# maxwerhahn/Multi-pass-GAN

Hardware: AMD Instinct MI355X
Metric: volumes/sec (4x two-pass generator inference, 64^3->256^3 density-only) (higher is better)
Workload: dtype f16+2xbf6->f32

## Files before the change

multi-pass-gan_amd/csrc/mpgan_conv.h:

```cpp
#pragma once
#include "mpgan_internal.h"
#include "mpgan_mfma_dev.h"

namespace mpg::conv {

using namespace mpg::dev;

constexpr int TW = 32;
constexpr int TAPOFF_BYTES = 1024;
constexpr int epi_rowf(int nt) { return nt * 32 + 4; }

struct SegArgs {
    const char* x;
    const char* w;
    int cg_seg;
    int cg_total, g_off;
    int kh, kw, up;
    int cgc, nchunks, sc;
    int ih, iw;
    int pt, pl;
    int hs, ws;
    int np;
    int ni_img;
    int direct;
// ... 51 lines not shown

template <int NT, int PREC>
struct Pipe {
    static constexpr int WAVES = 4;
    static constexpr int NPL = (PREC == 3) ? 2 : 1;
    static constexpr int PT = (NT >= 3) ? 2 : 4;
    static constexpr int TH = 4 * PT;
    static constexpr int KS = (PREC == 3) ? ((NT == 4 || NT == 2) ? 1 : 2) : ((NT == 4 || NT == 2) ? 2 : 4);
    static constexpr int R = (NT == 3) ? 3 : 4;
    static constexpr int D = R - 1;
    static constexpr int WPLANE = KS * NT * 1024;
    static constexpr int WSTAGE = WPLANE * NPL;
    static constexpr int NI = WSTAGE / 4096;
    static constexpr int ROWF = epi_rowf(NT);
    static_assert(WSTAGE % 4096 == 0, "stage must be a whole number of 256 x 16-byte pieces");
};

template <int NT>
struct Pipe6 {
    static constexpr int WAVES = (NT == 1) ? 4 : 8;
    static constexpr int PT = 16 / WAVES;
    static constexpr int TH = 16;
    static constexpr int KS = 4;
    static constexpr int WF16 = KS * NT * 1024;
    static constexpr int WF6 = NT * 2048;
    static constexpr int WSTAGE = WF16 + 2 * WF6;
    static constexpr int R = 3;
    static constexpr int D = R - 1;
    static constexpr int NI = WSTAGE / (WAVES * 1024);
    static constexpr int ROWF = epi_rowf(NT);
    static_assert(WSTAGE % (WAVES * 1024) == 0, "stage must be a whole number of per-wave pieces");
};

template <int NT, int PT, bool D2S = false>
__device__ __forceinline__ void conv_epilogue(f32x16 (&acc)[PT][NT], const KArgs ap, char* smem, int n, int y0, int x0,
                                              int wave, int lane) {
    const auto& a = *ap;
    const KArgsD2S dp = reinterpret_cast<KArgsD2S>(ap);
    const int r = lane & 31;
    const int hh = lane >> 5;
    constexpr int ROWF = epi_rowf(NT);
    float* stg = reinterpret_cast<float*>(smem + TAPOFF_BYTES) + wave * (32 * ROWF);
    const int cg_out = (a.cout + 7) >> 3;
    const float unscale = a.in_amax != nullptr ? 1.f / mpg::pow2_scale(*a.in_amax) : 1.f;
#pragma unroll
    for (int pt = 0; pt < PT; ++pt) {
        const int py = y0 + PT * wave + pt;
        float ss = 0.f;
#pragma unroll
        for (int nt = 0; nt < NT; ++nt)
#pragma unroll
            for (int q4 = 0; q4 < 4; ++q4) {
                const int co0 = nt * 32 + 8 * q4 + 4 * hh;
                float b4[4] = {0.f, 0.f, 0.f, 0.f};
                if (a.bias != nullptr) {
#pragma unroll
                    for (int i = 0; i < 4; ++i)
                        if (co0 + i < a.cout) b4[i] = a.bias[co0 + i];
                }
#pragma unroll
                for (int i = 0; i < 4; ++i) {
                    float v = mpg::apply_act(acc[pt][nt][4 * q4 + i] * unscale + b4[i], a.act, a.leak);
                    if (co0 + i >= a.cout) v = 0.f;
                    acc[pt][nt][4 * q4 + i] = v;
                    ss += v * v;
                }
            }
        if (a.pn) {
            ss += __shfl_xor(ss, 32);
            const float sc = rsqrtf(ss / (float)a.cout + a.pn_eps);
#pragma unroll
            for (int nt = 0; nt < NT; ++nt)
#pragma unroll
                for (int i = 0; i < 16; ++i) acc[pt][nt][i] *= sc;
        }
        if (a.y == nullptr && a.post_add == nullptr) {
            const int npx = min(32, a.w - x0);
            if (py < a.h && r < npx && !(a.dbg & 2)) {
                const size_t plane_px = (size_t)a.h * a.w;
#pragma unroll
                for (int nt = 0; nt < NT; ++nt)
#pragma unroll
                    for (int qp = 0; qp < 2; ++qp) {
                        float v[8];
#pragma unroll
                        for (int i = 0; i < 4; ++i) {
                            typedef unsigned v2u_t __attribute__((ext_vector_type(2)));
                            const v2u_t sw = __builtin_amdgcn_permlane32_swap(__float_as_uint(acc[pt][nt][8 * qp + i]),
                                                                              __float_as_uint(acc[pt][nt][8 * qp + 4 + i]), false, false);
                            v[i] = __uint_as_float(sw[0]);
                            v[4 + i] = __uint_as_float(sw[1]);
                        }
                        const int cg = nt * 4 + 2 * qp + hh;
                        if (cg < cg_out) {
                            char* dst;
                            size_t plane_out = plane_px;
                            if constexpr (D2S) {
                                const D2SPos q = d2s_pos(dp, py, x0 + r, 8 * cg);
                                plane_out = 4 * plane_px;
                                dst = a.y_g8 + ((((size_t)n * dp->cg + (q.cc >> 3)) * 2) * plane_out + q.pix) * 16;
                            } else {
                                dst = a.y_g8 + ((((size_t)n * cg_out + cg) * 2) * plane_px + (size_t)py * a.w + x0 + r) * 16;
                            }
                            half8 hi, lo;
#pragma unroll
                            for (int j = 0; j < 8; ++j) {
                                hi[j] = (_Float16)v[j];
                                lo[j] = (_Float16)(v[j] - (float)hi[j]);
                            }
                            __builtin_nontemporal_store(hi, reinterpret_cast<half8*>(dst));
                            __builtin_nontemporal_store(lo, reinterpret_cast<half8*>(dst + plane_out * 16));
                        }
                    }
            }
            continue;
        }
#pragma unroll
        for (int nt = 0; nt < NT; ++nt)
#pragma unroll
            for (int q4 = 0; q4 < 4; ++q4) {
                const int co0 = nt * 32 + 8 * q4 + 4 * hh;
                *reinterpret_cast<float4*>(stg + r * ROWF + co0) =
                    make_float4(acc[pt][nt][4 * q4], acc[pt][nt][4 * q4 + 1], acc[pt][nt][4 * q4 + 2], acc[pt][nt][4 * q4 + 3]);
            }
        if (py < a.h && !(a.dbg & 2)) {
            const int npx = min(32, a.w - x0);
            const size_t pix0 = ((size_t)n * a.h + py) * a.w + x0;
            if (a.post_add != nullptr) {
                const float* pa = a.post_add + pix0 * a.pa_stride + a.pa_coff;
                for (int f = lane; f < npx * a.cout; f += 64) {
                    const int p = f / a.cout;
                    const int c = f - p * a.cout;
                    stg[p * ROWF + c] += pa[(size_t)p * a.pa_stride + c];
                }
            }
            if (D2S && a.y != nullptr) {
                float* img = a.y + (size_t)n * 4 * a.h * a.w * dp->cs;
                const int total = npx * a.cout;
                if (((dp->cs | dp->coff | a.cout) & 3) == 0) {
                    for (int f = lane * 4; f < total; f += 256) {
                        const int p = f / a.cout;
                        const int c = f - p * a.cout;
                        const D2SPos q = d2s_pos(dp, py, x0 + p, c);
                        *reinterpret_cast<float4*>(img + q.pix * dp->cs + q.cc) = *reinterpret_cast<const float4*>(stg + p * ROWF + c);
                    }
                } else {
                    for (int f = lane; f < total; f += 64) {
                        const int p = f / a.cout;
                        const int c = f - p * a.cout;
                        const D2SPos q = d2s_pos(dp, py, x0 + p, c);
                        img[q.pix * dp->cs + q.cc] = stg[p * ROWF + c];
                    }
                }
            } else if (a.y != nullptr) {
                float* dst = a.y + pix0 * a.cout;
                const int total = npx * a.cout;
                if ((a.cout & 3) == 0) {
                    for (int f = lane * 4; f < total; f += 256) {
                        const int p = f / a.cout;
                        const int c = f - p * a.cout;
                        *reinterpret_cast<float4*>(dst + f) = *reinterpret_cast<const float4*>(stg + p * ROWF + c);
                    }
                } else {
                    for (int f = lane; f < total; f += 64) {
                        const int p = f / a.cout;
                        dst[f] = stg[p * ROWF + (f - p * a.cout)];
                    }
                }
            }
            if (a.y_g8 != nullptr) {
                const size_t plane_px = (size_t)a.h * a.w;
                if (r < npx) {
                    for (int cg = hh; cg < cg_out; cg += 2) {
                        const float4 v0 = *reinterpret_cast<const float4*>(stg + r * ROWF + cg * 8);
                        const float4 v1 = *reinterpret_cast<const float4*>(stg + r * ROWF + cg * 8 + 4);
                        const float v[8] = {v0.x, v0.y, v0.z, v0.w, v1.x, v1.y, v1.z, v1.w};
                        char* dst;
                        size_t plane_out = plane_px;
                        if constexpr (D2S) {
                            const D2SPos q = d2s_pos(dp, py, x0 + r, 8 * cg);
                            plane_out = 4 * plane_px;
                            dst = a.y_g8 + ((((size_t)n * dp->cg + (q.cc >> 3)) * 2) * plane_out + q.pix) * 16;
                        } else {
                            dst = a.y_g8 + ((((size_t)n * cg_out + cg) * 2) * plane_px + (size_t)py * a.w + x0 + r) * 16;
                        }
                        half8 hi, lo;
#pragma unroll
                        for (int j = 0; j < 8; ++j) {
                            hi[j] = (_Float16)v[j];
                            lo[j] = (_Float16)(v[j] - (float)hi[j]);
                        }
                        __builtin_nontemporal_store(hi, reinterpret_cast<half8*>(dst));
                        __builtin_nontemporal_store(lo, reinterpret_cast<half8*>(dst + plane_out * 16));
                    }
                }
            }
        }
    }
}

struct Shape {
    int th;
    int ks;
    int waves;
// ... 27 lines not shown
```

multi-pass-gan_amd/csrc/mpgan_conv_f16.hip:

```cpp
#include "mpgan_conv.h"

using namespace mpg::conv;

namespace {

template <int NT, int PREC, bool D2S = false>
__global__ __launch_bounds__(256, (NT >= 2 ? 2 : 3)) void conv_mfma_kernel(const typename KernelArgs<D2S>::type a_unused) {
    extern __shared__ __attribute__((aligned(16))) char smem[];
    const KArgs ap = (KArgs)__builtin_amdgcn_kernarg_segment_ptr();
    const auto& a = *ap;
    using P = Pipe<NT, PREC>;
    constexpr int PT = P::PT, TH = P::TH, KS = P::KS, WPLANE = P::WPLANE, WSTAGE = P::WSTAGE;
    constexpr int NI = P::NI, R = P::R, D = P::D;

    int* tapoff = reinterpret_cast<int*>(smem);
    char* img_lds = smem + TAPOFF_BYTES;
    char* w_lds = img_lds + 2 * a.img_bytes;

    const int tid = threadIdx.x;
    const int lane = tid & 63;
    const int wave = tid >> 6;
    const int wave_u = __builtin_amdgcn_readfirstlane(wave);
    const int r = lane & 31;
    const int hh = lane >> 5;

    int bid = blockIdx.x;
    const int nblk = gridDim.x;
    if ((nblk & 7) == 0) bid = (bid & 7) * (nblk >> 3) + (bid >> 3);
    const int tx = bid % a.tiles_x;
    const int t2 = bid / a.tiles_x;
    const int ty = t2 % a.tiles_y;
    const int n = t2 / a.tiles_y;
    const int y0 = ty * TH, x0 = tx * TW;

    f32x16 acc[PT][NT];
#pragma unroll
    for (int pt = 0; pt < PT; ++pt)
#pragma unroll
        for (int nt = 0; nt < NT; ++nt)
#pragma unroll
            for (int i = 0; i < 16; ++i) acc[pt][nt][i] = 0.f;

    for (int s = 0; s < ((a.dbg & 1) ? 0 : a.nseg); ++s) {
        const auto& sg = ap->seg[s];
        const int CGC = sg.cgc;
        const int TG = sg.kh * sg.kw * CGC;
        const int plane_b = sg.np * 16;
        const int group_b = plane_b * 2;
        const int ppg = sg.np >> 6;

        for (int q = tid; q < sg.sc * KS * 2; q += 256) {
            int off = 0;
            if (q < TG) {
                const int tap = q / CGC;
                const int g = q - tap * CGC;
                const int dy = tap / sg.kw;
                const int dx = tap - dy * sg.kw;
                off = (dy * sg.iw + dx) * 16 + g * group_b;
            }
            tapoff[q] = off;
        }
        int pixb[PT];
#pragma unroll
        for (int pt = 0; pt < PT; ++pt) pixb[pt] = ((PT * wave + pt) * sg.iw + r) * 16;

        const size_t plane_px = (size_t)sg.hs * sg.ws;
        auto dma_image = [&](int chunk) {
            char* buf = img_lds + (chunk & 1) * a.img_bytes;
            for (int i = 0; i < sg.ni_img; ++i) {
                const int pc = 4 * i + wave_u;
                const int g = pc / (2 * ppg);
                const int rem = pc - g * 2 * ppg;
                const int pl = rem / ppg;
                const int p = (rem - pl * ppg) * 64 + lane;
                const int hy = p / sg.iw;
// ... 33 lines not shown
                const char* wb = w_lds + (gst % R) * WSTAGE;
#pragma unroll
                for (int ks = 0; ks < KS; ++ks) {
                    const int toff = tapoff[2 * (st * KS + ks) + hh];
                    half8 b_hi[PT], b_lo[PT], a_hi[NT], a_lo[NT];
#pragma unroll
                    for (int pt = 0; pt < PT; ++pt) {
                        b_hi[pt] = *reinterpret_cast<const half8*>(img + pixb[pt] + toff);
                        if (PREC == 3) b_lo[pt] = *reinterpret_cast<const half8*>(img + plane_b + pixb[pt] + toff);
                    }
#pragma unroll
                    for (int nt = 0; nt < NT; ++nt) {
                        a_hi[nt] = *reinterpret_cast<const half8*>(wb + ((ks * NT + nt) * 64 + lane) * 16);
                        if (PREC == 3)
                            a_lo[nt] = *reinterpret_cast<const half8*>(wb + WPLANE + ((ks * NT + nt) * 64 + lane) * 16);
                    }
#pragma unroll
                    for (int nt = 0; nt < NT; ++nt)
#pragma unroll
                        for (int pt = 0; pt < PT; ++pt) {
                            acc[pt][nt] = __builtin_amdgcn_mfma_f32_32x32x16_f16(a_hi[nt], b_hi[pt], acc[pt][nt], 0, 0, 0);
                            if (PREC == 3) {
                                acc[pt][nt] = __builtin_amdgcn_mfma_f32_32x32x16_f16(a_lo[nt], b_hi[pt], acc[pt][nt], 0, 0, 0);
                                acc[pt][nt] = __builtin_amdgcn_mfma_f32_32x32x16_f16(a_hi[nt], b_lo[pt], acc[pt][nt], 0, 0, 0);
                            }
                        }
                }
            }
        }
        asm volatile("s_waitcnt vmcnt(0)" ::: "memory");
        __syncthreads();
    }

    conv_epilogue<NT, PT, D2S>(acc, ap, smem, n, y0, x0, wave, lane);
}

template <bool D2S>
hipError_t launch(int prec, int nt, dim3 grid, size_t lds, hipStream_t st, const typename KernelArgs<D2S>::type& a) {
    const dim3 block(256);
    if (prec == MPG_PREC_F16X3) {
        switch (nt) {
            case 1: return mpg::launch_dyn_lds<conv_mfma_kernel<1, 3, D2S>>(grid, block, lds, st, a);
            case 2: return mpg::launch_dyn_lds<conv_mfma_kernel<2, 3, D2S>>(grid, block, lds, st, a);
            case 3: return mpg::launch_dyn_lds<conv_mfma_kernel<3, 3, D2S>>(grid, block, lds, st, a);
            default: return mpg::launch_dyn_lds<conv_mfma_kernel<4, 3, D2S>>(grid, block, lds, st, a);
        }
    }
    switch (nt) {
        case 1: return mpg::launch_dyn_lds<conv_mfma_kernel<1, 1, D2S>>(grid, block, lds, st, a);
        case 2: return mpg::launch_dyn_lds<conv_mfma_kernel<2, 1, D2S>>(grid, block, lds, st, a);
        case 3: return mpg::launch_dyn_lds<conv_mfma_kernel<3, 1, D2S>>(grid, block, lds, st, a);
        default: return mpg::launch_dyn_lds<conv_mfma_kernel<4, 1, D2S>>(grid, block, lds, st, a);
    }
}

}

hipError_t mpg::conv::launch_conv_f16(int prec, int nt, dim3 grid, size_t lds, hipStream_t st, const ConvArgs& a) {
    return launch<false>(prec, nt, grid, lds, st, a);
}
hipError_t mpg::conv::launch_conv_f16(int prec, int nt, dim3 grid, size_t lds, hipStream_t st, const ConvArgsD2S& a) {
    return launch<true>(prec, nt, grid, lds, st, a);
}
```

multi-pass-gan_amd/csrc/mpgan_conv_f6.hip:

```cpp
#include "mpgan_conv.h"

using namespace mpg::conv;

namespace {

#ifndef MPG_AH
#define MPG_AH 2
#endif
#ifndef MPG_WD
#define MPG_WD 1
#endif
#ifndef MPG_DIAG6
#define MPG_DIAG6 0
#endif
#ifndef MPG_W0
#define MPG_W0 1
#endif
#ifndef MPG_IMG_LATE
#define MPG_IMG_LATE 0
#endif
#ifndef MPG_PIECES_AFTER
#define MPG_PIECES_AFTER 1
#endif
#ifndef MPG_ALT
// ... 85 lines not shown
    const auto& a = *ap;
    using P = Pipe6<NT>;
    constexpr int WAVES = P::WAVES, PT = P::PT, TH = P::TH, WF16 = P::WF16, WF6 = P::WF6, WSTAGE = P::WSTAGE;
    constexpr int NI = P::NI, R = P::R, D = P::D, THREADS = WAVES * 64;

    int* tap16 = reinterpret_cast<int*>(smem);
    char* img_lds = smem + a.tap_bytes;
    char* w_lds = img_lds + 2 * a.img_bytes;

    const int tid = threadIdx.x;
    const int lane = tid & 63;
    const int wave = tid >> 6;
    const int wave_u = __builtin_amdgcn_readfirstlane(wave);
    const int r = lane & 31;
    const int hh = lane >> 5;

    int bid = blockIdx.x;
    const int nblk = gridDim.x;
    if ((nblk & 7) == 0) bid = (bid & 7) * (nblk >> 3) + (bid >> 3);
    const int tx = bid % a.tiles_x;
    const int t2 = bid / a.tiles_x;
    const int ty = t2 % a.tiles_y;
    const int n = t2 / a.tiles_y;
    const int y0 = ty * TH, x0 = tx * TW;

    f32x16 acc[PT][NT];
#pragma unroll
    for (int pt = 0; pt < PT; ++pt)
#pragma unroll
        for (int nt = 0; nt < NT; ++nt)
#pragma unroll
            for (int i = 0; i < 16; ++i) acc[pt][nt][i] = 0.f;

    const int seg_flip = (NT == 1 && a.nseg > 1) ? ((int)(blockIdx.x >> 8) & 1) : 0;
    for (int s0 = 0; s0 < ((a.dbg & 1) ? 0 : a.nseg); ++s0) {
        const int s = seg_flip ? a.nseg - 1 - s0 : s0;
        const auto& sg = ap->seg[s];
        if (NT <= 2 && sg.direct) {
            const unsigned plane_bytes = (unsigned)(sg.hs * sg.ws) * 16u;
            const unsigned gstride = 2u * plane_bytes;
            const char* xb = sg.x + ((size_t)n * sg.cg_total + sg.g_off) * gstride;
            unsigned pixo[PT];
#pragma unroll
            for (int pt = 0; pt < PT; ++pt) {
                int yy = y0 + PT * wave + pt, xx = x0 + r;
                yy = (yy < a.h ? yy : a.h - 1) >> sg.up;
                xx = (xx < a.w ? xx : a.w - 1) >> sg.up;
                pixo[pt] = (unsigned)(yy * sg.ws + xx) * 16u;
            }
            const int glast = sg.cg_seg - 1;
            auto dma_stage_d = [&](int stage) {
                const int sidx = stage < sg.sc ? stage : sg.sc - 1;
                const char* src = sg.w + (size_t)sidx * WSTAGE + tid * 16;
                char* dst = w_lds + (stage % R) * WSTAGE + wave_u * 1024;
#pragma unroll
                for (int i = 0; i < NI; ++i) dma16(src + i * (THREADS * 16), dst + i * (THREADS * 16));
            };
#pragma unroll
            for (int d = 0; d < D; ++d) dma_stage_d(d);
            for (int st = 0; st < sg.sc; ++st) {
                wait_dma_and_barrier<(D - 1) * NI>();
                dma_stage_d(st + D);
                const char* wb = w_lds + (st % R) * WSTAGE;
                const char* xs = xb + (size_t)st * 8 * gstride;
                const int grem = glast - st * 8;
                constexpr int PH = PT == 4 ? 1 : 2;
// ... 286 lines not shown
                    });
                });
                lgkm_wait<0>();
                static_for<0, PT>([&](auto pc) {
                    static_for<0, 4>([&](auto jc) { tie(bh[decltype(pc)::value][decltype(jc)::value]); });
                    make_hi6(pc);
                });
                MPG_STAMP(ts1);
                bf6_phase(std::integral_constant<int, 0>{});
                MPG_STAMP(ts2);
                fp16_phase(std::integral_constant<int, 0>{});
            } else {
                fp16_phase(std::integral_constant<int, 1>{});
                MPG_STAMP(ts2);
                bf6_phase(std::integral_constant<int, MPG_W0>{});
            }
            MPG_STAMP(ts3);
        }
        };
#if MPG_ALT
        if (WAVES == 8 && wave_u >= WAVES / 2) run_stages(std::integral_constant<int, 1>{});
        else
#endif
            run_stages(std::integral_constant<int, 0>{});
        asm volatile("s_waitcnt vmcnt(0) lgkmcnt(0)" ::: "memory");
        __syncthreads();
#if MPG_STAMPS
        if ((a.dbg & 8) && a.y != nullptr && s == 0 && lane == 0) {
            unsigned* o = reinterpret_cast<unsigned*>(a.y) + ((size_t)blockIdx.x * WAVES + wave) * 4;
            o[0] = sum_head; o[1] = sum_f16; o[2] = sum_f6; o[3] = sum_bar;
        }
#endif
    }
    conv_epilogue<NT, PT>(acc, ap, smem, n, y0, x0, wave, lane);
}

}

hipError_t mpg::conv::launch_conv_f6(int nt, dim3 grid, size_t lds, hipStream_t st, const ConvArgs& a) {
    switch (nt) {
        case 1: return mpg::launch_dyn_lds<conv_mfma_f6_kernel<1>>(grid, dim3(Pipe6<1>::WAVES * 64), lds, st, a);
        case 2: return mpg::launch_dyn_lds<conv_mfma_f6_kernel<2>>(grid, dim3(Pipe6<2>::WAVES * 64), lds, st, a);
        case 3: return mpg::launch_dyn_lds<conv_mfma_f6_kernel<3>>(grid, dim3(Pipe6<3>::WAVES * 64), lds, st, a);
        default: return mpg::launch_dyn_lds<conv_mfma_f6_kernel<4>>(grid, dim3(Pipe6<4>::WAVES * 64), lds, st, a);
    }
}
```

multi-pass-gan_amd/csrc/mpgan_conv_small.hip:

```cpp
#include "mpgan_conv.h"

using namespace mpg::conv;

namespace {

#ifndef MPG_SM_PAD
#define MPG_SM_PAD 0
#endif

struct SmallSeg {
    const char* x;
    const float* w;
    int cg_total, g_off, kh, kw, up, pt, pl, hs, ws, cin;
};

struct SmallArgs {
    int n, h, w, cout, nseg;
    int tile_floats;
    SmallSeg seg[MPG_MAX_SEG];
    const float* bias;
    const float* in_amax;
    int act;
    float leak;
    float* y;
    char* y_g8;
};

__device__ __forceinline__ void g8_load8(const char* src, size_t plane_bytes, float (&v)[8]) {
    const half8 hi = *reinterpret_cast<const half8*>(src);
    const half8 lo = *reinterpret_cast<const half8*>(src + plane_bytes);
#pragma unroll
    for (int j = 0; j < 8; ++j) v[j] = (float)hi[j] + (float)lo[j];
}

#ifndef MPG_SM_RPT
#define MPG_SM_RPT 4
#endif
constexpr int SM_TW = 64, SM_RPT = MPG_SM_RPT, SM_TH = 4 * SM_RPT, SM_KMAX = 7;
#ifndef MPG_DIAG_SMALL
#define MPG_DIAG_SMALL 0
#endif
#ifndef MPG_SMALL_INV
#define MPG_SMALL_INV 0
#endif
#if MPG_DIAG_SMALL
__device__ unsigned g_small_diag[2];
#endif

template <int COUT, int CINB>
__global__ __launch_bounds__(256) void conv_small_kernel(SmallArgs a) {
    extern __shared__ __attribute__((aligned(16))) float small_lds[];
    constexpr int PL = (CINB + 3) / 4;
    constexpr int CP = CINB < 4 ? CINB : 4;
    float4* tile = reinterpret_cast<float4*>(small_lds);
    float* wl = small_lds + a.tile_floats;
    const int tid = threadIdx.x;
    const int lx = tid % SM_TW, yg = tid / SM_TW;
    const int x0 = blockIdx.x * SM_TW, y0 = blockIdx.y * SM_TH, b = blockIdx.z;
#if MPG_SMALL_INV
    asm volatile("buffer_inv sc0 sc1" ::: "memory");
#endif
    float acc[SM_RPT][COUT];
#pragma unroll
    for (int j = 0; j < SM_RPT; ++j)
#pragma unroll
        for (int co = 0; co < COUT; ++co) acc[j][co] = 0.f;
    for (int s = 0; s < a.nseg; ++s) {
        const SmallSeg& g = a.seg[s];
        const size_t plane_bytes = (size_t)g.hs * g.ws * 16;
        const char* base = g.x + ((size_t)b * g.cg_total + g.g_off) * 2 * plane_bytes;
        const int tw = SM_TW + g.kw - 1, th = SM_TH + g.kh - 1;
        if (s > 0) __syncthreads();
        for (int p = tid; p < g.kh * g.kw * CINB * COUT; p += 256) {
            const int co = p % COUT, ci = (p / COUT) % CINB, tap = p / (COUT * CINB);
            wl[p] = g.w[tap * 64 + ci * 8 + co];
        }
        for (int p = tid; p < tw * th; p += 256) {
            const int hy = p / tw, hx = p - hy * tw;
            const int yy = y0 - g.pt + hy, xx = x0 - g.pl + hx;
            float v[8];
            if (yy >= 0 && yy < a.h && xx >= 0 && xx < a.w) {
                g8_load8(base + ((size_t)(yy >> g.up) * g.ws + (xx >> g.up)) * 16, plane_bytes, v);
            } else {
#pragma unroll
                for (int q = 0; q < 8; ++q) v[q] = 0.f;
            }
            tile[p] = make_float4(v[0], v[1], v[2], v[3]);
            if (PL > 1) tile[th * tw + p] = make_float4(v[4], v[5], v[6], v[7]);
        }
        __syncthreads();
        const int kh = g.kh;
        for (int kx = 0; kx < g.kw; ++kx) {
            float rows[SM_RPT + SM_KMAX - 1][CINB];
#pragma unroll
// ... 38 lines not shown
            }
        }
#if MPG_DIAG_SMALL
        {
            __syncthreads();
            unsigned bad_w = 0, bad_t = 0;
            for (int p = tid; p < g.kh * g.kw * CINB * COUT; p += 256) {
                const int co = p % COUT, ci = (p / COUT) % CINB, tap = p / (COUT * CINB);
                if (wl[p] != g.w[tap * 64 + ci * 8 + co]) ++bad_w;
            }
            for (int p = tid; p < tw * th; p += 256) {
                const int hy = p / tw, hx = p - hy * tw;
                const int yy = y0 - g.pt + hy, xx = x0 - g.pl + hx;
                float v[8];
                if (yy >= 0 && yy < a.h && xx >= 0 && xx < a.w) {
                    g8_load8(base + ((size_t)(yy >> g.up) * g.ws + (xx >> g.up)) * 16, plane_bytes, v);
                } else {
                    for (int q = 0; q < 8; ++q) v[q] = 0.f;
                }
                const float4 t0 = tile[p];
                if (t0.x != v[0] || t0.y != v[1] || t0.z != v[2] || t0.w != v[3]) ++bad_t;
                if (PL > 1) {
                    const float4 t1 = tile[th * tw + p];
                    if (t1.x != v[4] || t1.y != v[5] || t1.z != v[6] || t1.w != v[7]) ++bad_t;
                }
            }
            if (bad_w) atomicAdd(&g_small_diag[0], bad_w);
            if (bad_t) atomicAdd(&g_small_diag[1], bad_t);
        }
#endif
    }
    const int x = x0 + lx;
    if (x >= a.w) return;
    const float unscale = a.in_amax != nullptr ? 1.f / mpg::pow2_scale(*a.in_amax) : 1.f;
    const size_t plane_px = (size_t)a.h * a.w;
#pragma unroll
    for (int j = 0; j < SM_RPT; ++j) {
        const int y = y0 + yg * SM_RPT + j;
        if (y >= a.h) break;
        float o[8];
#pragma unroll
        for (int q = 0; q < 8; ++q)
            o[q] = (q < COUT && q < a.cout) ? mpg::apply_act(acc[j][q < COUT ? q : 0] * unscale + (a.bias != nullptr ? a.bias[q] : 0.f),
                                                              a.act, a.leak)
                                            : 0.f;
        const size_t pix = (size_t)y * a.w + x;
        if (a.y != nullptr) {
            float* dst = a.y + ((size_t)b * plane_px + pix) * a.cout;
#pragma unroll
            for (int q = 0; q < 8; ++q)
                if (q < a.cout) dst[q] = o[q];
        }
        if (a.y_g8 != nullptr) {
            half8 hi, lo;
#pragma unroll
            for (int q = 0; q < 8; ++q) {
                hi[q] = (_Float16)o[q];
                lo[q] = (_Float16)(o[q] - (float)hi[q]);
            }
            char* dst = a.y_g8 + ((size_t)b * 2 * plane_px + pix) * 16;
            *reinterpret_cast<half8*>(dst) = hi;
            *reinterpret_cast<half8*>(dst + plane_px * 16) = lo;
        }
    }
}

struct PairArgs {
    int n, h, w;
    const char* x;
    int cg_total, g_off, up, hs, ws;
    const float *wa, *wb, *wsc;
    int kha, kwa, pta, pla;
    int khb, kwb, ptb, plb;
    int khs, kws, pts, pls;
    const float *bias_a, *bias_b;
    int act_a, act_b;
    float leak_a, leak_b;
    int cout;
    float* y;
    char* y_g8;
    int x_px, mid_px;
};

template <int CINB, int COUTB>
__device__ __forceinline__ void small_column(const float4* tile, int tw, int plane_px, int row0, int col, const float* wl,
                                             int kh, int kw, float (&acc)[SM_RPT][COUTB]) {
    constexpr int PL = (CINB + 3) / 4, CP = CINB < 4 ? CINB : 4;
    for (int kx = 0; kx < kw; ++kx) {
        float rows[SM_RPT + SM_KMAX - 1][CINB];
#pragma unroll
        for (int r = 0; r < SM_RPT + SM_KMAX - 1; ++r) {
            if (r < SM_RPT + kh - 1) {
                const float4* src = tile + (row0 + r) * tw + col + kx;
                const float4 p0 = src[0];
                rows[r][0] = p0.x;
                if constexpr (CP > 1) rows[r][1] = p0.y;
                if constexpr (CP > 2) { rows[r][2] = p0.z; rows[r][3] = p0.w; }
                if constexpr (PL > 1) {
                    const float4 p1 = src[plane_px];
                    rows[r][4] = p1.x; rows[r][5] = p1.y; rows[r][6] = p1.z; rows[r][7] = p1.w;
                }
            }
        }
#pragma unroll
        for (int ky = 0; ky < SM_KMAX; ++ky) {
            if (ky < kh) {
                const float* wt = wl + (ky * kw + kx) * (CINB * COUTB);
#pragma unroll
                for (int ci = 0; ci < CINB; ++ci) {
                    float wv[COUTB];
#pragma unroll
                    for (int co = 0; co < COUTB; ++co) wv[co] = wt[ci * COUTB + co];
#pragma unroll
                    for (int j = 0; j < SM_RPT; ++j)
#pragma unroll
                        for (int co = 0; co < COUTB; ++co) acc[j][co] = fmaf(rows[j + ky][ci], wv[co], acc[j][co]);
                }
            }
        }
    }
}

template <int CINB, int CMIDB, int COUTB>
__global__ __launch_bounds__(256) void conv_small_pair_kernel(PairArgs a) {
    extern __shared__ __attribute__((aligned(16))) float small_lds[];
    constexpr int PLX = (CINB + 3) / 4, PLM = (CMIDB + 3) / 4;
    float4* xt = reinterpret_cast<float4*>(small_lds);
    float4* mt = xt + PLX * a.x_px;
    float* wla = reinterpret_cast<float*>(mt + PLM * a.mid_px);
    float* wlb = wla + a.kha * a.kwa * CINB * CMIDB;
    float* wls = wlb + a.khb * a.kwb * CMIDB * COUTB;
    const int tid = threadIdx.x;
    const int x0 = blockIdx.x * SM_TW, y0 = blockIdx.y * SM_TH, b = blockIdx.z;
    const int mw = SM_TW + a.kwb - 1, mh = SM_TH + a.khb - 1;
    const int xw = mw + a.kwa - 1, xh = mh + a.kha - 1;
    const int mx0 = x0 - a.plb, my0 = y0 - a.ptb;
    const int xx0 = mx0 - a.pla, xy0 = my0 - a.pta;
    for (int p = tid; p < a.kha * a.kwa * CINB * CMIDB; p += 256) {
        const int co = p % CMIDB, ci = (p / CMIDB) % CINB, tap = p / (CMIDB * CINB);
        wla[p] = a.wa[tap * 64 + ci * 8 + co];
    }
    for (int p = tid; p < a.khb * a.kwb * CMIDB * COUTB; p += 256) {
        const int co = p % COUTB, ci = (p / COUTB) % CMIDB, tap = p / (COUTB * CMIDB);
        wlb[p] = a.wb[tap * 64 + ci * 8 + co];
    }
    if (a.wsc != nullptr)
        for (int p = tid; p < a.khs * a.kws * CINB * COUTB; p += 256) {
            const int co = p % COUTB, ci = (p / COUTB) % CINB, tap = p / (COUTB * CINB);
            wls[p] = a.wsc[tap * 64 + ci * 8 + co];
        }
    {
        const size_t plane_bytes = (size_t)a.hs * a.ws * 16;
        const char* base = a.x + ((size_t)b * a.cg_total + a.g_off) * 2 * plane_bytes;
        for (int p = tid; p < xw * xh; p += 256) {
            const int hy = p / xw, hx = p - hy * xw;
            const int yy = xy0 + hy, xx = xx0 + hx;
            float v[8];
            if (yy >= 0 && yy < a.h && xx >= 0 && xx < a.w) {
                g8_load8(base + ((size_t)(yy >> a.up) * a.ws + (xx >> a.up)) * 16, plane_bytes, v);
            } else {
#pragma unroll
                for (int q = 0; q < 8; ++q) v[q] = 0.f;
            }
            xt[p] = make_float4(v[0], v[1], v[2], v[3]);
            if (PLX > 1) xt[a.x_px + p] = make_float4(v[4], v[5], v[6], v[7]);
        }
    }
    __syncthreads();
    const int mgroups = (mh + SM_RPT - 1) / SM_RPT;
    for (int t = tid; t < mw * mgroups; t += 256) {
        const int col = t % mw, rg = t / mw;
        float acc[SM_RPT][CMIDB];
#pragma unroll
        for (int j = 0; j < SM_RPT; ++j)
#pragma unroll
            for (int c = 0; c < CMIDB; ++c) acc[j][c] = 0.f;
        small_column<CINB, CMIDB>(xt, xw, a.x_px, rg * SM_RPT, col, wla, a.kha, a.kwa, acc);
#pragma unroll
        for (int j = 0; j < SM_RPT; ++j) {
            const int row = rg * SM_RPT + j;
            if (row < mh) {
                const int yy = my0 + row, xx = mx0 + col;
                const bool in = yy >= 0 && yy < a.h && xx >= 0 && xx < a.w;
                float o[8];
#pragma unroll
                for (int c = 0; c < 8; ++c)
                    o[c] = (c < CMIDB && in) ? mpg::apply_act(acc[j][c < CMIDB ? c : 0] + (a.bias_a != nullptr ? a.bias_a[c] : 0.f), a.act_a, a.leak_a) : 0.f;
                mt[row * mw + col] = make_float4(o[0], o[1], o[2], o[3]);
                if (PLM > 1) mt[a.mid_px + row * mw + col] = make_float4(o[4], o[5], o[6], o[7]);
            }
        }
    }
    __syncthreads();
    const int lx = tid % SM_TW, yg = tid / SM_TW;
    float acc[SM_RPT][COUTB];
#pragma unroll
    for (int j = 0; j < SM_RPT; ++j)
#pragma unroll
        for (int c = 0; c < COUTB; ++c) acc[j][c] = 0.f;
    small_column<CMIDB, COUTB>(mt, mw, a.mid_px, yg * SM_RPT, lx, wlb, a.khb, a.kwb, acc);
    if (a.wsc != nullptr)
        small_column<CINB, COUTB>(xt, xw, a.x_px, yg * SM_RPT + a.ptb + a.pta - a.pts, lx + a.plb + a.pla - a.pls, wls, a.khs, a.kws, acc);
    const int x = x0 + lx;
    if (x >= a.w) return;
    const size_t plane_px = (size_t)a.h * a.w;
#pragma unroll
    for (int j = 0; j < SM_RPT; ++j) {
        const int y = y0 + yg * SM_RPT + j;
        if (y >= a.h) break;
        float o[8];
#pragma unroll
        for (int q = 0; q < 8; ++q)
            o[q] = (q < COUTB && q < a.cout) ? mpg::apply_act(acc[j][q < COUTB ? q : 0] + (a.bias_b != nullptr ? a.bias_b[q] : 0.f), a.act_b, a.leak_b) : 0.f;
        const size_t pix = (size_t)y * a.w + x;
        if (a.y != nullptr) {
            float* dst = a.y + ((size_t)b * plane_px + pix) * a.cout;
#pragma unroll
            for (int q = 0; q < 8; ++q)
                if (q < a.cout) dst[q] = o[q];
        }
        if (a.y_g8 != nullptr) {
            half8 hi, lo;
#pragma unroll
            for (int q = 0; q < 8; ++q) {
                hi[q] = (_Float16)o[q];
                lo[q] = (_Float16)(o[q] - (float)hi[q]);
            }
            char* dst = a.y_g8 + ((size_t)b * 2 * plane_px + pix) * 16;
            *reinterpret_cast<half8*>(dst) = hi;
            *reinterpret_cast<half8*>(dst + plane_px * 16) = lo;
        }
    }
}

}

int mpg::conv::launch_small(hipStream_t stream, const mpg_conv_desc* d) {
    SmallArgs sa;
    sa.n = d->n; sa.h = d->h; sa.w = d->w; sa.cout = d->cout; sa.nseg = d->nseg;
    int cmax = 1, tmax = 1, tile_px = 0;
    for (int s = 0; s < d->nseg; ++s) {
        if (const int rc = check_segment(d, s)) return rc;
        const mpg_conv_seg& g = d->seg[s];
        SmallSeg& o = sa.seg[s];
        o.x = (const char*)g.x;
        o.w = (const float*)((const char*)g.wpack + pack_base_bytes(g.kh, g.kw, g.cin, d->cout, d->prec));
        o.cg_total = g.cgroups; o.g_off = g.g_off; o.kh = g.kh; o.kw = g.kw; o.up = g.up_log2;
        o.pt = pad_before(g.kh, g.pad_hi); o.pl = pad_before(g.kw, g.pad_hi);
        o.hs = d->h >> g.up_log2; o.ws = d->w >> g.up_log2; o.cin = g.cin;
        cmax = g.cin > cmax ? g.cin : cmax;
        tmax = g.kh * g.kw > tmax ? g.kh * g.kw : tmax;
        const int px = (SM_TH + g.kh - 1) * (SM_TW + g.kw - 1);
        tile_px = px > tile_px ? px : tile_px;
    }
    for (int s = d->nseg; s < MPG_MAX_SEG; ++s) sa.seg[s] = sa.seg[0];
    sa.bias = d->bias; sa.in_amax = d->in_amax; sa.act = d->act; sa.leak = d->leak;
    sa.y = d->y; sa.y_g8 = (char*)d->y_g8;
    MPG_REQUIRE((((uintptr_t)d->y_g8) & 15) == 0, "mpg_conv2d_fused: misaligned output");
    const dim3 grid((unsigned)((d->w + SM_TW - 1) / SM_TW), (unsigned)((d->h + SM_TH - 1) / SM_TH), (unsigned)d->n);
// ... 14 lines not shown
    MPG_LAUNCH_CHECK("conv_small_kernel");
}

extern "C" int mpg_conv2d_small_pair(mpg_stream_t stream, const mpg_small_pair_desc* d) {
    MPG_REQUIRE(d != nullptr, "mpg_conv2d_small_pair: null desc");
    MPG_REQUIRE(d->n >= 1 && d->h >= 1 && d->w >= 1 && d->n <= 65535, "mpg_conv2d_small_pair: bad shape %d x %d x %d", d->n, d->h, d->w);
    MPG_REQUIRE(d->cin >= 1 && d->cin <= 8 && d->cmid >= 1 && d->cmid <= 8 && d->cout >= 1 && d->cout <= 8,
                "mpg_conv2d_small_pair: %d -> %d -> %d channels (1..8 each)", d->cin, d->cmid, d->cout);
    MPG_REQUIRE(d->x && d->wpack_a && d->wpack_b, "mpg_conv2d_small_pair: null pointer");
    MPG_REQUIRE(d->y != nullptr || d->y_g8 != nullptr, "mpg_conv2d_small_pair: no output requested");
    MPG_REQUIRE(d->kh_a >= 1 && d->kh_a <= 7 && d->kw_a >= 1 && d->kw_a <= 7 && d->kh_b >= 1 && d->kh_b <= 7 && d->kw_b >= 1 && d->kw_b <= 7,
                "mpg_conv2d_small_pair: kernel sizes 1..7");
    MPG_REQUIRE((d->kh_a & 1) && (d->kw_a & 1) && (d->kh_b & 1) && (d->kw_b & 1), "mpg_conv2d_small_pair: odd filters only");
    MPG_REQUIRE(d->wpack_s == nullptr || (d->kh_s >= 1 && d->kh_s <= d->kh_a + d->kh_b - 1 && d->kw_s >= 1 && d->kw_s <= d->kw_a + d->kw_b - 1 &&
                                          (d->kh_s & 1) && (d->kw_s & 1) && ((d->kh_a + d->kh_b) & 1) == 0 && ((d->kw_a + d->kw_b) & 1) == 0),
                "mpg_conv2d_small_pair: the shortcut filter must be odd and fit inside the input tile of two odd filters");
    MPG_REQUIRE(d->g_off >= 0 && d->g_off < d->cgroups, "mpg_conv2d_small_pair: channel-group range");
    MPG_REQUIRE(d->up_log2 >= 0 && d->up_log2 <= 4 && (d->h % (1 << d->up_log2)) == 0 && (d->w % (1 << d->up_log2)) == 0,
                "mpg_conv2d_small_pair: upsample %d", d->up_log2);
    MPG_REQUIRE(d->act_a >= MPG_ACT_NONE && d->act_a <= MPG_ACT_TANH && d->act_b >= MPG_ACT_NONE && d->act_b <= MPG_ACT_TANH, "mpg_conv2d_small_pair: bad act");
    MPG_REQUIRE(d->prec == MPG_PREC_F16X1 || d->prec == MPG_PREC_F16X3 || d->prec == MPG_PREC_F16F6, "mpg_conv2d_small_pair: bad prec %d", d->prec);
    MPG_REQUIRE((((uintptr_t)d->x) & 15) == 0 && (((uintptr_t)d->y_g8) & 15) == 0, "mpg_conv2d_small_pair: misaligned tensor");
    PairArgs a;
    a.n = d->n; a.h = d->h; a.w = d->w;
    a.x = (const char*)d->x; a.cg_total = d->cgroups; a.g_off = d->g_off; a.up = d->up_log2;
    a.hs = d->h >> d->up_log2; a.ws = d->w >> d->up_log2;
    a.wa = (const float*)((const char*)d->wpack_a + pack_base_bytes(d->kh_a, d->kw_a, d->cin, d->cmid, d->prec));
    a.wb = (const float*)((const char*)d->wpack_b + pack_base_bytes(d->kh_b, d->kw_b, d->cmid, d->cout, d->prec));
    a.wsc = d->wpack_s ? (const float*)((const char*)d->wpack_s + pack_base_bytes(d->kh_s, d->kw_s, d->cin, d->cout, d->prec)) : nullptr;
    a.kha = d->kh_a; a.kwa = d->kw_a; a.pta = pad_before(d->kh_a, 0); a.pla = pad_before(d->kw_a, 0);
    a.khb = d->kh_b; a.kwb = d->kw_b; a.ptb = pad_before(d->kh_b, 0); a.plb = pad_before(d->kw_b, 0);
    a.khs = d->wpack_s ? d->kh_s : 1; a.kws = d->wpack_s ? d->kw_s : 1; a.pts = pad_before(a.khs, 0); a.pls = pad_before(a.kws, 0);
    a.bias_a = d->bias_a; a.bias_b = d->bias_b; a.act_a = d->act_a; a.act_b = d->act_b; a.leak_a = d->leak_a; a.leak_b = d->leak_b;
    a.cout = d->cout; a.y = d->y; a.y_g8 = (char*)d->y_g8;
    const int mw = SM_TW + a.kwb - 1, mh = SM_TH + a.khb - 1;
    const int mgroups = (mh + SM_RPT - 1) / SM_RPT;
    const int xw = mw + a.kwa - 1, xh = mgroups * SM_RPT + a.kha - 1;
    a.x_px = xw * xh;
    a.mid_px = mw * (mgroups * SM_RPT + a.khb - 1);
    const int ci = d->cin == 1 ? 1 : d->cin <= 4 ? 4 : 8, cm = d->cmid <= 2 ? 2 : 8, co = d->cout == 1 ? 1 : 8;
    const size_t lds = ((size_t)((ci + 3) / 4) * a.x_px + (size_t)((cm + 3) / 4) * a.mid_px) * 16 +
                       ((size_t)a.kha * a.kwa * ci * cm + (size_t)a.khb * a.kwb * cm * co + (size_t)a.khs * a.kws * ci * co) * sizeof(float);
    MPG_REQUIRE(lds <= LDS_MAX, "mpg_conv2d_small_pair: LDS budget %zu exceeds 160 KiB", lds);
    const dim3 grid((unsigned)((d->w + SM_TW - 1) / SM_TW), (unsigned)((d->h + SM_TH - 1) / SM_TH), (unsigned)d->n);
    hipError_t le = hipSuccess;
    switch (ci * 100 + cm * 10 + co) {
#define MPG_PAIR(CI, CM, CO) case CI * 100 + CM * 10 + CO: \
        le = mpg::launch_dyn_lds<conv_small_pair_kernel<CI, CM, CO>>(grid, dim3(256), lds, (hipStream_t)stream, a); break;
        MPG_PAIR(1, 2, 1) MPG_PAIR(1, 2, 8) MPG_PAIR(1, 8, 1) MPG_PAIR(1, 8, 8)
        MPG_PAIR(4, 2, 1) MPG_PAIR(4, 2, 8) MPG_PAIR(4, 8, 1) MPG_PAIR(4, 8, 8)
        MPG_PAIR(8, 2, 1) MPG_PAIR(8, 2, 8) MPG_PAIR(8, 8, 1) MPG_PAIR(8, 8, 8)
#undef MPG_PAIR
        default: break;
    }
    if (le != hipSuccess) return mpg::hip_check(le, "mpg_conv2d_small_pair: hipFuncSetAttribute(dynamic LDS)");
    MPG_LAUNCH_CHECK("conv_small_pair_kernel");
}

#if MPG_DIAG_SMALL
extern "C" int mpg_debug_small_diag(unsigned* out2) {
    return hipMemcpyFromSymbol(out2, HIP_SYMBOL(g_small_diag), 8) == hipSuccess ? 0 : 1;
}
#endif
```

Before: 14.25.

## Prefetch bias and amax before main loop, stage bias in LDS, specialize activation

Bias values and the input amax scale are now loaded at kernel start, before the conv main loop, so their global-memory latency is hidden. The bias is staged into LDS and read back as float4, replacing scalar per-element global loads in the epilogue. The activation function is specialized at compile time through a switch, and tanh is run as a non-unrolled loop over an LDS staging row. The post-add loop issues four loads before its stores. The small kernels get the same bias hoisting and activation specialization. In exchange the epilogue gains an extra __syncthreads, more live registers, and one instantiation per activation type.

Measured after the change: 15.28, median of 6. +7.2%, better.

```diff
diff --git a/multi-pass-gan_amd/csrc/mpgan_conv.h b/multi-pass-gan_amd/csrc/mpgan_conv.h
--- a/multi-pass-gan_amd/csrc/mpgan_conv.h
+++ b/multi-pass-gan_amd/csrc/mpgan_conv.h
@@ -107,52 +107,126 @@
     static_assert(WSTAGE % (WAVES * 1024) == 0, "stage must be a whole number of per-wave pieces");
 };
 
+struct EpiPre {
+    float bias;
+    float amax;
+};
+__device__ __forceinline__ EpiPre epilogue_prefetch(const KArgs ap, int tid) {
+    const auto& a = *ap;
+    EpiPre pre;
+    pre.bias = (a.bias != nullptr && tid < a.cout) ? a.bias[tid] : 0.f;
+    pre.amax = a.in_amax != nullptr ? *a.in_amax : 0.f;
+    return pre;
+}
+
+template <int ACT, int NT>
+__device__ __forceinline__ void epilogue_bias_act(f32x16 (&acc)[NT], const float* bl, float* stg_lane, float unscale, float leak, int cout,
+                                                  int hh) {
+    if constexpr (ACT == MPG_ACT_TANH) {
+#pragma unroll
+        for (int nt = 0; nt < NT; ++nt)
+#pragma unroll
+            for (int q4 = 0; q4 < 4; ++q4) {
+                const int co0 = nt * 32 + 8 * q4 + 4 * hh;
+                const float4 bq = *reinterpret_cast<const float4*>(bl + co0);
+                *reinterpret_cast<float4*>(stg_lane + co0) =
+                    make_float4(acc[nt][4 * q4] * unscale + bq.x, acc[nt][4 * q4 + 1] * unscale + bq.y,
+                                acc[nt][4 * q4 + 2] * unscale + bq.z, acc[nt][4 * q4 + 3] * unscale + bq.w);
+            }
+#pragma nounroll
+        for (int k = 0; k < NT * 16; ++k) {
+            const int c = (k >> 2) * 8 + 4 * hh + (k & 3);
+            stg_lane[c] = c < cout ? tanhf(stg_lane[c]) : 0.f;
+        }
+#pragma unroll
+        for (int nt = 0; nt < NT; ++nt)
+#pragma unroll
+            for (int q4 = 0; q4 < 4; ++q4) {
+                const float4 v = *reinterpret_cast<const float4*>(stg_lane + nt * 32 + 8 * q4 + 4 * hh);
+                acc[nt][4 * q4] = v.x;
+                acc[nt][4 * q4 + 1] = v.y;
+                acc[nt][4 * q4 + 2] = v.z;
+                acc[nt][4 * q4 + 3] = v.w;
+            }
+        return;
+    }
+    float4 bq[2][4];
+#pragma unroll
+    for (int q4 = 0; q4 < 4; ++q4) bq[0][q4] = *reinterpret_cast<const float4*>(bl + 8 * q4 + 4 * hh);
+#pragma unroll
+    for (int nt = 0; nt < NT; ++nt) {
+        if (nt + 1 < NT) {
+#pragma unroll
+            for (int q4 = 0; q4 < 4; ++q4) bq[(nt + 1) & 1][q4] = *reinterpret_cast<const float4*>(bl + (nt + 1) * 32 + 8 * q4 + 4 * hh);
+        }
+        __builtin_amdgcn_sched_barrier(0);
+#pragma unroll
+        for (int q4 = 0; q4 < 4; ++q4) {
+            const int co0 = nt * 32 + 8 * q4 + 4 * hh;
+            const float b4[4] = {bq[nt & 1][q4].x, bq[nt & 1][q4].y, bq[nt & 1][q4].z, bq[nt & 1][q4].w};
+#pragma unroll
+            for (int i = 0; i < 4; ++i) {
+                float v = mpg::apply_act(acc[nt][4 * q4 + i] * unscale + b4[i], ACT, leak);
+                if (co0 + i >= cout) v = 0.f;
+                acc[nt][4 * q4 + i] = v;
+            }
+        }
+        __builtin_amdgcn_sched_barrier(0);
+    }
+}
+
+template <int NT>
+__device__ __forceinline__ void epilogue_row_values(f32x16 (&acc)[NT], const KArgs ap, const float* bl, float* stg_lane, float unscale,
+                                                    int hh) {
+    const auto& a = *ap;
+    switch (a.act) {
+        case MPG_ACT_RELU: epilogue_bias_act<MPG_ACT_RELU>(acc, bl, stg_lane, unscale, a.leak, a.cout, hh); break;
+        case MPG_ACT_LRELU: epilogue_bias_act<MPG_ACT_LRELU>(acc, bl, stg_lane, unscale, a.leak, a.cout, hh); break;
+        case MPG_ACT_TANH: epilogue_bias_act<MPG_ACT_TANH>(acc, bl, stg_lane, unscale, a.leak, a.cout, hh); break;
+        default: epilogue_bias_act<MPG_ACT_NONE>(acc, bl, stg_lane, unscale, a.leak, a.cout, hh); break;
+    }
+    if (a.pn) {
+        float ss = 0.f;
+#pragma unroll
+        for (int nt = 0; nt < NT; ++nt)
+#pragma unroll
+            for (int i = 0; i < 16; ++i) ss += acc[nt][i] * acc[nt][i];
+        ss += __shfl_xor(ss, 32);
+        const float sc = rsqrtf(ss / (float)a.cout + a.pn_eps);
+#pragma unroll
+        for (int nt = 0; nt < NT; ++nt)
+#pragma unroll
+            for (int i = 0; i < 16; ++i) acc[nt][i] *= sc;
+    }
+}
+
 template <int NT, int PT, bool D2S = false>
 __device__ __forceinline__ void conv_epilogue(f32x16 (&acc)[PT][NT], const KArgs ap, char* smem, int n, int y0, int x0,
-                                              int wave, int lane) {
+                                              int wave, int lane, const EpiPre pre) {
     const auto& a = *ap;
     const KArgsD2S dp = reinterpret_cast<KArgsD2S>(ap);
     const int r = lane & 31;
     const int hh = lane >> 5;
     constexpr int ROWF = epi_rowf(NT);
+    static_assert(128 * sizeof(float) <= TAPOFF_BYTES, "the staged bias must fit in front of the staging rows");
+    float* bl = reinterpret_cast<float*>(smem);
     float* stg = reinterpret_cast<float*>(smem + TAPOFF_BYTES) + wave * (32 * ROWF);
     const int cg_out = (a.cout + 7) >> 3;
-    const float unscale = a.in_amax != nullptr ? 1.f / mpg::pow2_scale(*a.in_amax) : 1.f;
-#pragma unroll
-    for (int pt = 0; pt < PT; ++pt) {
-        const int py = y0 + PT * wave + pt;
-        float ss = 0.f;
-#pragma unroll
-        for (int nt = 0; nt < NT; ++nt)
-#pragma unroll
-            for (int q4 = 0; q4 < 4; ++q4) {
-                const int co0 = nt * 32 + 8 * q4 + 4 * hh;
-                float b4[4] = {0.f, 0.f, 0.f, 0.f};
-                if (a.bias != nullptr) {
-#pragma unroll
-                    for (int i = 0; i < 4; ++i)
-                        if (co0 + i < a.cout) b4[i] = a.bias[co0 + i];
-                }
-#pragma unroll
-                for (int i = 0; i < 4; ++i) {
-                    float v = mpg::apply_act(acc[pt][nt][4 * q4 + i] * unscale + b4[i], a.act, a.leak);
-                    if (co0 + i >= a.cout) v = 0.f;
-                    acc[pt][nt][4 * q4 + i] = v;
-                    ss += v * v;
-                }
-            }
-        if (a.pn) {
-            ss += __shfl_xor(ss, 32);
-            const float sc = rsqrtf(ss / (float)a.cout + a.pn_eps);
-#pragma unroll
-            for (int nt = 0; nt < NT; ++nt)
-#pragma unroll
-                for (int i = 0; i < 16; ++i) acc[pt][nt][i] *= sc;
-        }
-        if (a.y == nullptr && a.post_add == nullptr) {
-            const int npx = min(32, a.w - x0);
+    const float unscale = 1.f / mpg::pow2_scale(pre.amax);
+    {
+        float bv = pre.bias;
+        asm volatile("" : "+v"(bv));
+        if (wave < 2) bl[wave * 64 + lane] = bv;
+    }
+    __syncthreads();
+    const int npx = min(32, a.w - x0);
+    const size_t plane_px = (size_t)a.h * a.w;
+    if (a.y == nullptr && a.post_add == nullptr) {
+#pragma unroll
+        for (int pt = 0; pt < PT; ++pt) {
+            const int py = y0 + PT * wave + pt;
+            epilogue_row_values<NT>(acc[pt], ap, bl, stg + r * ROWF, unscale, hh);
             if (py < a.h && r < npx && !(a.dbg & 2)) {
-                const size_t plane_px = (size_t)a.h * a.w;
 #pragma unroll
                 for (int nt = 0; nt < NT; ++nt)
 #pragma unroll
@@ -188,8 +262,13 @@
                         }
                     }
             }
-            continue;
-        }
+        }
+        return;
+    }
+#pragma unroll
+    for (int pt = 0; pt < PT; ++pt) {
+        const int py = y0 + PT * wave + pt;
+        epilogue_row_values<NT>(acc[pt], ap, bl, stg + r * ROWF, unscale, hh);
 #pragma unroll
         for (int nt = 0; nt < NT; ++nt)
 #pragma unroll
@@ -199,14 +278,26 @@
                     make_float4(acc[pt][nt][4 * q4], acc[pt][nt][4 * q4 + 1], acc[pt][nt][4 * q4 + 2], acc[pt][nt][4 * q4 + 3]);
             }
         if (py < a.h && !(a.dbg & 2)) {
-            const int npx = min(32, a.w - x0);
             const size_t pix0 = ((size_t)n * a.h + py) * a.w + x0;
             if (a.post_add != nullptr) {
                 const float* pa = a.post_add + pix0 * a.pa_stride + a.pa_coff;
-                for (int f = lane; f < npx * a.cout; f += 64) {
-                    const int p = f / a.cout;
-                    const int c = f - p * a.cout;
-                    stg[p * ROWF + c] += pa[(size_t)p * a.pa_stride + c];
+                const int total = npx * a.cout;
+                for (int f0 = lane; f0 < total; f0 += 256) {
+                    float pv[4];
+                    int so[4];
+#pragma unroll
+                    for (int j = 0; j < 4; ++j) {
+                        const int f = min(f0 + 64 * j, total - 1);
+                        const int p = f / a.cout;
+                        const int c = f - p * a.cout;
+                        so[j] = p * ROWF + c;
+                        pv[j] = pa[(size_t)p * a.pa_stride + c];
+                    }
+#pragma unroll
+                    for (int j = 0; j < 4; ++j) {
+                        asm volatile("" : "+v"(pv[j]));
+                        if (f0 + 64 * j < total) stg[so[j]] += pv[j];
+                    }
                 }
             }
             if (D2S && a.y != nullptr) {
@@ -244,7 +335,6 @@
                 }
             }
             if (a.y_g8 != nullptr) {
-                const size_t plane_px = (size_t)a.h * a.w;
                 if (r < npx) {
                     for (int cg = hh; cg < cg_out; cg += 2) {
                         const float4 v0 = *reinterpret_cast<const float4*>(stg + r * ROWF + cg * 8);
diff --git a/multi-pass-gan_amd/csrc/mpgan_conv_f16.hip b/multi-pass-gan_amd/csrc/mpgan_conv_f16.hip
--- a/multi-pass-gan_amd/csrc/mpgan_conv_f16.hip
+++ b/multi-pass-gan_amd/csrc/mpgan_conv_f16.hip
@@ -41,6 +41,7 @@
 #pragma unroll
             for (int i = 0; i < 16; ++i) acc[pt][nt][i] = 0.f;
 
+    const EpiPre pre = epilogue_prefetch(ap, tid);
     for (int s = 0; s < ((a.dbg & 1) ? 0 : a.nseg); ++s) {
         const auto& sg = ap->seg[s];
         const int CGC = sg.cgc;
@@ -140,7 +141,7 @@
         __syncthreads();
     }
 
-    conv_epilogue<NT, PT, D2S>(acc, ap, smem, n, y0, x0, wave, lane);
+    conv_epilogue<NT, PT, D2S>(acc, ap, smem, n, y0, x0, wave, lane, pre);
 }
 
 template <bool D2S>
diff --git a/multi-pass-gan_amd/csrc/mpgan_conv_f6.hip b/multi-pass-gan_amd/csrc/mpgan_conv_f6.hip
--- a/multi-pass-gan_amd/csrc/mpgan_conv_f6.hip
+++ b/multi-pass-gan_amd/csrc/mpgan_conv_f6.hip
@@ -141,6 +141,7 @@
 #pragma unroll
             for (int i = 0; i < 16; ++i) acc[pt][nt][i] = 0.f;
 
+    const EpiPre pre = epilogue_prefetch(ap, tid);
     const int seg_flip = (NT == 1 && a.nseg > 1) ? ((int)(blockIdx.x >> 8) & 1) : 0;
     for (int s0 = 0; s0 < ((a.dbg & 1) ? 0 : a.nseg); ++s0) {
         const int s = seg_flip ? a.nseg - 1 - s0 : s0;
@@ -493,7 +494,7 @@
         }
 #endif
     }
-    conv_epilogue<NT, PT>(acc, ap, smem, n, y0, x0, wave, lane);
+    conv_epilogue<NT, PT>(acc, ap, smem, n, y0, x0, wave, lane, pre);
 }
 
 }
diff --git a/multi-pass-gan_amd/csrc/mpgan_conv_small.hip b/multi-pass-gan_amd/csrc/mpgan_conv_small.hip
--- a/multi-pass-gan_amd/csrc/mpgan_conv_small.hip
+++ b/multi-pass-gan_amd/csrc/mpgan_conv_small.hip
@@ -46,6 +46,25 @@
 #if MPG_DIAG_SMALL
 __device__ unsigned g_small_diag[2];
 #endif
+
+template <int C>
+__device__ __forceinline__ void small_bias(const float* bias, int cout, float (&bq)[C]) {
+#pragma unroll
+    for (int q = 0; q < C; ++q) bq[q] = 0.f;
+    if (bias != nullptr) {
+#pragma unroll
+        for (int q = 0; q < C; ++q) bq[q] = bias[q < cout ? q : cout - 1];
+    }
+}
+template <class F>
+__device__ __forceinline__ void with_act(int act, F&& f) {
+    switch (act) {
+        case MPG_ACT_RELU: f(std::integral_constant<int, MPG_ACT_RELU>{}); break;
+        case MPG_ACT_LRELU: f(std::integral_constant<int, MPG_ACT_LRELU>{}); break;
+        case MPG_ACT_TANH: f(std::integral_constant<int, MPG_ACT_TANH>{}); break;
+        default: f(std::integral_constant<int, MPG_ACT_NONE>{}); break;
+    }
+}
 
 template <int COUT, int CINB>
 __global__ __launch_bounds__(256) void conv_small_kernel(SmallArgs a) {
@@ -60,6 +79,9 @@
 #if MPG_SMALL_INV
     asm volatile("buffer_inv sc0 sc1" ::: "memory");
 #endif
+    float bq[COUT];
+    small_bias(a.bias, a.cout, bq);
+    const float amax = a.in_amax != nullptr ? *a.in_amax : 0.f;
     float acc[SM_RPT][COUT];
 #pragma unroll
     for (int j = 0; j < SM_RPT; ++j)
@@ -164,31 +186,34 @@
     }
     const int x = x0 + lx;
     if (x >= a.w) return;
-    const float unscale = a.in_amax != nullptr ? 1.f / mpg::pow2_scale(*a.in_amax) : 1.f;
+    const float unscale = 1.f / mpg::pow2_scale(amax);
     const size_t plane_px = (size_t)a.h * a.w;
+    float o[SM_RPT][8];
+    with_act(a.act, [&](auto actc) {
+        constexpr int ACT = decltype(actc)::value;
+#pragma unroll
+        for (int j = 0; j < SM_RPT; ++j)
+#pragma unroll
+            for (int q = 0; q < 8; ++q)
+                o[j][q] = (q < COUT && q < a.cout) ? mpg::apply_act(acc[j][q < COUT ? q : 0] * unscale + bq[q < COUT ? q : 0], ACT, a.leak) : 0.f;
+    });
 #pragma unroll
     for (int j = 0; j < SM_RPT; ++j) {
         const int y = y0 + yg * SM_RPT + j;
         if (y >= a.h) break;
-        float o[8];
-#pragma unroll
-        for (int q = 0; q < 8; ++q)
-            o[q] = (q < COUT && q < a.cout) ? mpg::apply_act(acc[j][q < COUT ? q : 0] * unscale + (a.bias != nullptr ? a.bias[q] : 0.f),
-                                                              a.act, a.leak)
-                                            : 0.f;
         const size_t pix = (size_t)y * a.w + x;
         if (a.y != nullptr) {
             float* dst = a.y + ((size_t)b * plane_px + pix) * a.cout;
 #pragma unroll
             for (int q = 0; q < 8; ++q)
-                if (q < a.cout) dst[q] = o[q];
+                if (q < a.cout) dst[q] = o[j][q];
         }
         if (a.y_g8 != nullptr) {
             half8 hi, lo;
 #pragma unroll
             for (int q = 0; q < 8; ++q) {
-                hi[q] = (_Float16)o[q];
-                lo[q] = (_Float16)(o[q] - (float)hi[q]);
+                hi[q] = (_Float16)o[j][q];
+                lo[q] = (_Float16)(o[j][q] - (float)hi[q]);
             }
             char* dst = a.y_g8 + ((size_t)b * 2 * plane_px + pix) * 16;
             *reinterpret_cast<half8*>(dst) = hi;
@@ -208,7 +233,7 @@
     const float *bias_a, *bias_b;
     int act_a, act_b;
     float leak_a, leak_b;
-    int cout;
+    int cmid, cout;
     float* y;
     char* y_g8;
     int x_px, mid_px;
@@ -264,6 +289,9 @@
     float* wls = wlb + a.khb * a.kwb * CMIDB * COUTB;
     const int tid = threadIdx.x;
     const int x0 = blockIdx.x * SM_TW, y0 = blockIdx.y * SM_TH, b = blockIdx.z;
+    float bqa[CMIDB], bqb[COUTB];
+    small_bias(a.bias_a, a.cmid, bqa);
+    small_bias(a.bias_b, a.cout, bqb);
     const int mw = SM_TW + a.kwb - 1, mh = SM_TH + a.khb - 1;
     const int xw = mw + a.kwa - 1, xh = mh + a.kha - 1;
     const int mx0 = x0 - a.plb, my0 = y0 - a.ptb;
@@ -308,18 +336,23 @@
 #pragma unroll
             for (int c = 0; c < CMIDB; ++c) acc[j][c] = 0.f;
         small_column<CINB, CMIDB>(xt, xw, a.x_px, rg * SM_RPT, col, wla, a.kha, a.kwa, acc);
+        float o[SM_RPT][8];
+        with_act(a.act_a, [&](auto actc) {
+            constexpr int ACT = decltype(actc)::value;
+#pragma unroll
+            for (int j = 0; j < SM_RPT; ++j)
+#pragma unroll
+                for (int c = 0; c < 8; ++c)
+                    o[j][c] = c < CMIDB ? mpg::apply_act(acc[j][c < CMIDB ? c : 0] + bqa[c < CMIDB ? c : 0], ACT, a.leak_a) : 0.f;
+        });
 #pragma unroll
         for (int j = 0; j < SM_RPT; ++j) {
             const int row = rg * SM_RPT + j;
             if (row < mh) {
                 const int yy = my0 + row, xx = mx0 + col;
                 const bool in = yy >= 0 && yy < a.h && xx >= 0 && xx < a.w;
-                float o[8];
-#pragma unroll
-                for (int c = 0; c < 8; ++c)
-                    o[c] = (c < CMIDB && in) ? mpg::apply_act(acc[j][c < CMIDB ? c : 0] + (a.bias_a != nullptr ? a.bias_a[c] : 0.f), a.act_a, a.leak_a) : 0.f;
-                mt[row * mw + col] = make_float4(o[0], o[1], o[2], o[3]);
-                if (PLM > 1) mt[a.mid_px + row * mw + col] = make_float4(o[4], o[5], o[6], o[7]);
+                mt[row * mw + col] = in ? make_float4(o[j][0], o[j][1], o[j][2], o[j][3]) : make_float4(0.f, 0.f, 0.f, 0.f);
+                if (PLM > 1) mt[a.mid_px + row * mw + col] = in ? make_float4(o[j][4], o[j][5], o[j][6], o[j][7]) : make_float4(0.f, 0.f, 0.f, 0.f);
             }
         }
     }
@@ -336,27 +369,32 @@
     const int x = x0 + lx;
     if (x >= a.w) return;
     const size_t plane_px = (size_t)a.h * a.w;
+    float o[SM_RPT][8];
+    with_act(a.act_b, [&](auto actc) {
+        constexpr int ACT = decltype(actc)::value;
+#pragma unroll
+        for (int j = 0; j < SM_RPT; ++j)
+#pragma unroll
+            for (int q = 0; q < 8; ++q)
+                o[j][q] = (q < COUTB && q < a.cout) ? mpg::apply_act(acc[j][q < COUTB ? q : 0] + bqb[q < COUTB ? q : 0], ACT, a.leak_b) : 0.f;
+    });
 #pragma unroll
     for (int j = 0; j < SM_RPT; ++j) {
         const int y = y0 + yg * SM_RPT + j;
         if (y >= a.h) break;
-        float o[8];
-#pragma unroll
-        for (int q = 0; q < 8; ++q)
-            o[q] = (q < COUTB && q < a.cout) ? mpg::apply_act(acc[j][q < COUTB ? q : 0] + (a.bias_b != nullptr ? a.bias_b[q] : 0.f), a.act_b, a.leak_b) : 0.f;
         const size_t pix = (size_t)y * a.w + x;
         if (a.y != nullptr) {
             float* dst = a.y + ((size_t)b * plane_px + pix) * a.cout;
 #pragma unroll
             for (int q = 0; q < 8; ++q)
-                if (q < a.cout) dst[q] = o[q];
+                if (q < a.cout) dst[q] = o[j][q];
         }
         if (a.y_g8 != nullptr) {
             half8 hi, lo;
 #pragma unroll
             for (int q = 0; q < 8; ++q) {
-                hi[q] = (_Float16)o[q];
-                lo[q] = (_Float16)(o[q] - (float)hi[q]);
+                hi[q] = (_Float16)o[j][q];
+                lo[q] = (_Float16)(o[j][q] - (float)hi[q]);
             }
             char* dst = a.y_g8 + ((size_t)b * 2 * plane_px + pix) * 16;
             *reinterpret_cast<half8*>(dst) = hi;
@@ -437,7 +475,7 @@
     a.khb = d->kh_b; a.kwb = d->kw_b; a.ptb = pad_before(d->kh_b, 0); a.plb = pad_before(d->kw_b, 0);
     a.khs = d->wpack_s ? d->kh_s : 1; a.kws = d->wpack_s ? d->kw_s : 1; a.pts = pad_before(a.khs, 0); a.pls = pad_before(a.kws, 0);
     a.bias_a = d->bias_a; a.bias_b = d->bias_b; a.act_a = d->act_a; a.act_b = d->act_b; a.leak_a = d->leak_a; a.leak_b = d->leak_b;
-    a.cout = d->cout; a.y = d->y; a.y_g8 = (char*)d->y_g8;
+    a.cmid = d->cmid; a.cout = d->cout; a.y = d->y; a.y_g8 = (char*)d->y_g8;
     const int mw = SM_TW + a.kwb - 1, mh = SM_TH + a.khb - 1;
     const int mgroups = (mh + SM_RPT - 1) / SM_RPT;
     const int xw = mw + a.kwa - 1, xh = mgroups * SM_RPT + a.kha - 1;
```
